# autonomousvision/unimatch

Measured on NVIDIA H100. Metric: image-pairs/sec @480x832 gmflow-scale2-refine6; EPE vs reference, higher is better.
Workload: dtype fp32

## Files before the change

### unimatch_b200/csrc/um_attention_tc.cu

```cuda
#include <math_constants.h>

#include "um_common.cuh"
#include "um_tc.cuh"

namespace um {

using namespace tc;

namespace {

constexpr int BM = 128, BN = 64;
constexpr int NTHREADS = 288;
constexpr int PRODUCER = 8;
constexpr uint32_t Q_BYTES = 4 * 16384;
constexpr uint32_t KV_STAGE_BYTES = 4 * 8192;
constexpr uint32_t OFF_Q = 0;
constexpr uint32_t OFF_K = OFF_Q + Q_BYTES;
constexpr uint32_t OFF_V = OFF_K + 2 * KV_STAGE_BYTES;
constexpr uint32_t OFF_X = OFF_V + 2 * KV_STAGE_BYTES;
constexpr uint32_t OFF_BAR = OFF_X + 1024;
constexpr uint32_t OFF_KREG = OFF_BAR + 256;
constexpr int MAX_LP = 2048;
constexpr uint32_t SMEM_BYTES = OFF_KREG + MAX_LP;
constexpr float SQRT_C = 11.313708498984761f;
constexpr float EXP_SCALE = 1.4426950408889634f / 11.313708498984761f;
constexpr float LAZY_THRESH = 8.0f / EXP_SCALE;

struct TcParams {
  float* out; long long ldo;
  int n_streams, kv_shift, lp;
  Geom g;
  const float* values; int vdim, value_mode, post_op;
  __half* out_split; long long split_plane;
};

__device__ __forceinline__ uint32_t pack_h2(__half a, __half b) {
  return (uint32_t)__half_as_ushort(a) | ((uint32_t)__half_as_ushort(b) << 16);
}

template <bool HAS_V>
__global__ void __launch_bounds__(NTHREADS, 1)
attn_tc_kernel(const __grid_constant__ CUtensorMap map_q, const __grid_constant__ CUtensorMap map_k,
               const __grid_constant__ CUtensorMap map_v, TcParams p) {
  extern __shared__ __align__(1024) uint8_t smem[];
  uint64_t* bars = reinterpret_cast<uint64_t*>(smem + OFF_BAR);
  uint64_t* q_full = bars + 0;
  uint64_t* k_full = bars + 1;
  uint64_t* k_empty = bars + 3;
  uint64_t* v_full = bars + 5;
  uint64_t* v_empty = bars + 7;
  int8_t* kreg = reinterpret_cast<int8_t*>(smem + OFF_KREG);

  const Geom g = p.g;
  const int warp = threadIdx.x >> 5, lane = threadIdx.x & 31;
  const int m0 = blockIdx.x * BM, win = blockIdx.y, n = blockIdx.z;
  const int nk = (n + p.kv_shift) % p.n_streams;
  const int nwin = g.nwin, lp = p.lp;
  const int T = (g.lw + BN - 1) / BN;
  const int planes = p.n_streams * nwin * lp;

  if (threadIdx.x == 0) {
    mbar_init(q_full, 1);
    for (int i = 0; i < 2; ++i) {
      mbar_init(k_full + i, 1); mbar_init(k_empty + i, 8);
      mbar_init(v_full + i, 1); mbar_init(v_empty + i, 8);
    }
    fence_barrier_init();
  }
  if (warp == PRODUCER && lane == 0) { tma_prefetch_desc(&map_q); tma_prefetch_desc(&map_k); tma_prefetch_desc(&map_v); }
  bool masked = false;
  if (g.mask_mode == UM_MASK_SWIN) {
    const int wy = win / g.kw, wx = win - wy * g.kw;
    masked = (g.sh > 0 && wy == g.kh - 1) || (g.sw > 0 && wx == g.kw - 1);
    if (masked)
      for (int t = threadIdx.x; t < g.lw; t += NTHREADS) {
        int yr, xr;
        window_token(g, win, t, &yr, &xr);
        kreg[t] = (int8_t)shift_region(g, yr, xr);
      }
  }
  __syncthreads();

  if (warp == PRODUCER) {
    const int qrow = (n * nwin + win) * lp + m0;
    if (elect_one()) {
      mbar_arrive_expect_tx(q_full, Q_BYTES);
#pragma unroll
      for (int part = 0; part < 2; ++part)
#pragma unroll
        for (int half = 0; half < 2; ++half)
          tma_load_2d(smem + OFF_Q + (part * 2 + half) * 16384, &map_q, q_full, half * 64, part * planes + qrow);
    }
    __syncwarp();
    const int krow = (nk * nwin + win) * lp;
    auto load_tile = [&](int j, const CUtensorMap* map, uint32_t off, uint64_t* full, uint64_t* empty) {
      const int s = j & 1;
      mbar_wait_inline(empty + s, ((j >> 1) & 1) ^ 1);
      if (elect_one()) {
        mbar_arrive_expect_tx(full + s, KV_STAGE_BYTES);
#pragma unroll
        for (int part = 0; part < 2; ++part)
#pragma unroll
          for (int half = 0; half < 2; ++half)
            tma_load_2d(smem + off + s * KV_STAGE_BYTES + (part * 2 + half) * 8192, map, full + s, half * 64,
                        part * planes + krow + j * BN);
      }
      __syncwarp();
    };
    load_tile(0, &map_k, OFF_K, k_full, k_empty);
    for (int j = 0; j < T; ++j) {
      if (j + 1 < T) load_tile(j + 1, &map_k, OFF_K, k_full, k_empty);
      if (HAS_V) load_tile(j, &map_v, OFF_V, v_full, v_empty);
    }
    return;
  }

  const int cw = warp;
  const int wg = cw >> 2;
  const int fr = wg * 64 + (cw & 3) * 16 + (lane >> 2);
  const int fc = 2 * (lane & 3);
  int rq[2] = {0, 0}, tok[2];
  bool row_valid[2];
#pragma unroll
  for (int h = 0; h < 2; ++h) {
    const int tq = m0 + fr + 8 * h;
    row_valid[h] = tq < g.lw;
    int yr = 0, xr = 0;
    tok[h] = row_valid[h] ? window_token(g, win, tq, &yr, &xr) : -1;
    if (masked) rq[h] = shift_region(g, yr, xr);
  }
  float m_run[2] = {-CUDART_INF_F, -CUDART_INF_F}, l_run[2] = {0.f, 0.f};
  const uint32_t q_base = smem_u32(smem + OFF_Q) + wg * 8192;
  auto consumers_sync = [&]() { asm volatile("bar.sync 1, 256;" ::: "memory"); };

  auto compute_s = [&](int j, float (&sv)[32]) {
    const int s = j & 1;
    mbar_wait_inline(k_full + s, (j >> 1) & 1);
    const uint32_t k_base = smem_u32(smem + OFF_K + s * KV_STAGE_BYTES);
    const int qa[3] = {1, 0, 0}, kb[3] = {0, 1, 0};
    fence_acc(sv);
    wgmma_fence();
#pragma unroll
    for (int c = 0; c < 3; ++c)
#pragma unroll
      for (int half = 0; half < 2; ++half)
#pragma unroll
        for (int ks = 0; ks < 4; ++ks)
          wgmma_ss<BN>(sv, desc_kmajor(q_base + (qa[c] * 2 + half) * 16384 + ks * 32),
                       desc_kmajor(k_base + (kb[c] * 2 + half) * 8192 + ks * 32), (c | half | ks) != 0);
    wgmma_commit();
    wgmma_wait<0>();
    fence_acc(sv);
    __syncwarp();
    if (lane == 0) mbar_arrive(k_empty + s);
  };
  mbar_wait_inline(q_full, 0);

  if (!HAS_V) {
    float* vals = reinterpret_cast<float*>(smem + OFF_X);
    const int et = threadIdx.x;
    const long long L = (long long)g.h * g.w;
    float a0[2] = {0.f, 0.f}, a1[2] = {0.f, 0.f};
    for (int j = 0; j < T; ++j) {
      const int s = j & 1;
      const int n0 = j * BN;
      if (et < BN) {
        float v0 = 0.f, v1 = 0.f;
        const int t = n0 + et;
        if (t < g.lw) {
          const int ktok = window_token(g, win, t);
          if (p.value_mode == UM_VALUE_TENSOR) {
            const float* vp = p.values + ((long long)nk * L + ktok) * p.vdim;
            v0 = __ldg(vp); v1 = (p.vdim > 1) ? __ldg(vp + 1) : 0.f;
          } else {
            const int ky = ktok / g.w;
            v0 = (float)(ktok - ky * g.w); v1 = (float)ky;
          }
        }
        vals[(s * BN + et) * 2] = v0; vals[(s * BN + et) * 2 + 1] = v1;
      }
      float sv[32];
      compute_s(j, sv);
      consumers_sync();
      const float2* vv = reinterpret_cast<const float2*>(vals + s * BN * 2);
#pragma unroll
      for (int h = 0; h < 2; ++h) {
        float mx = -CUDART_INF_F;
#pragma unroll
        for (int jj = 0; jj < 8; ++jj)
#pragma unroll
          for (int e = 0; e < 2; ++e) {
            float& x = sv[4 * jj + 2 * h + e];
            if (n0 + 8 * jj + fc + e >= g.lw) x = -CUDART_INF_F;
            mx = fmaxf(mx, x);
          }
        mx = fmaxf(mx, __shfl_xor_sync(0xffffffffu, mx, 1));
        mx = fmaxf(mx, __shfl_xor_sync(0xffffffffu, mx, 2));
        const float m_new = fmaxf(m_run[h], mx);
        const float alpha = exp2f((m_run[h] - m_new) * EXP_SCALE);
        m_run[h] = m_new;
        const float mscaled = m_new * EXP_SCALE;
        float sum = 0.f, b0 = 0.f, b1 = 0.f;
#pragma unroll
        for (int jj = 0; jj < 8; ++jj)
#pragma unroll
          for (int e = 0; e < 2; ++e) {
            const float pe = ex2_approx(fmaf(sv[4 * jj + 2 * h + e], EXP_SCALE, -mscaled));
            const float2 kv = vv[8 * jj + fc + e];
            sum += pe;
            b0 = fmaf(pe, kv.x, b0);
            b1 = fmaf(pe, kv.y, b1);
          }
        l_run[h] = l_run[h] * alpha + sum;
        a0[h] = a0[h] * alpha + b0;
        a1[h] = a1[h] * alpha + b1;
      }
    }
#pragma unroll
    for (int h = 0; h < 2; ++h) {
#pragma unroll
      for (int o = 1; o <= 2; o <<= 1) {
        l_run[h] += __shfl_xor_sync(0xffffffffu, l_run[h], o);
        a0[h] += __shfl_xor_sync(0xffffffffu, a0[h], o);
        a1[h] += __shfl_xor_sync(0xffffffffu, a1[h], o);
      }
      if (row_valid[h] && (lane & 3) == 0) {
        float r0 = a0[h] / l_run[h], r1 = a1[h] / l_run[h];
        const int oy = tok[h] / g.w, ox = tok[h] - oy * g.w;
        if (p.post_op == UM_POST_MINUS_OWN) { r0 -= (float)ox; r1 -= (float)oy; }
        else if (p.post_op == UM_POST_OWN_MINUS) { r0 = (float)ox - r0; }
        float* dst = p.out + ((long long)n * L + tok[h]) * p.vdim;
        dst[0] = r0;
        if (p.vdim > 1) dst[1] = r1;
      }
    }
    return;
  }

  float o[64];
#pragma unroll
  for (int i = 0; i < 64; ++i) o[i] = 0.f;
  for (int j = 0; j < T; ++j) {
    const int s = j & 1;
    const int n0 = j * BN;
    float sv[32];
    compute_s(j, sv);
    uint32_t ph[16], pl[16];
#pragma unroll
    for (int h = 0; h < 2; ++h) {
#pragma unroll
      for (int jj = 0; jj < 8; ++jj)
#pragma unroll
        for (int e = 0; e < 2; ++e) {
          const int col = n0 + 8 * jj + fc + e;
          float& x = sv[4 * jj + 2 * h + e];
          if (masked && kreg[col < g.lw ? col : 0] != rq[h]) x -= 100.0f * SQRT_C;
          if (col >= g.lw) x = -CUDART_INF_F;
        }
      float mx = -CUDART_INF_F;
#pragma unroll
      for (int jj = 0; jj < 8; ++jj) mx = fmaxf(mx, fmaxf(sv[4 * jj + 2 * h], sv[4 * jj + 2 * h + 1]));
      mx = fmaxf(mx, __shfl_xor_sync(0xffffffffu, mx, 1));
      mx = fmaxf(mx, __shfl_xor_sync(0xffffffffu, mx, 2));
      float alpha = 1.0f;
      if (mx > m_run[h] + LAZY_THRESH) {
        alpha = exp2f((m_run[h] - mx) * EXP_SCALE);
        m_run[h] = mx;
#pragma unroll
        for (int jj = 0; jj < 16; ++jj) { o[4 * jj + 2 * h] *= alpha; o[4 * jj + 2 * h + 1] *= alpha; }
      }
      const float mscaled = m_run[h] * EXP_SCALE;
      float sum = 0.f;
#pragma unroll
      for (int jj = 0; jj < 8; ++jj) {
        const float p0 = ex2_approx(fmaf(sv[4 * jj + 2 * h], EXP_SCALE, -mscaled));
        const float p1 = ex2_approx(fmaf(sv[4 * jj + 2 * h + 1], EXP_SCALE, -mscaled));
        sum += p0 + p1;
        split_f16x2(p0, p1, &ph[2 * jj + h], &pl[2 * jj + h]);
      }
      l_run[h] = l_run[h] * alpha + sum;
    }
    mbar_wait_inline(v_full + s, (j >> 1) & 1);
    const uint32_t v_base = smem_u32(smem + OFF_V + s * KV_STAGE_BYTES);
    fence_acc(o);
    wgmma_fence();
#pragma unroll
    for (int c = 0; c < 3; ++c)
#pragma unroll
      for (int ks = 0; ks < 4; ++ks) {
        const uint32_t* pp = c == 0 ? pl : ph;
        const uint32_t a[4] = {pp[4 * ks], pp[4 * ks + 1], pp[4 * ks + 2], pp[4 * ks + 3]};
        wgmma_rs_n128_tb(o, a, desc_mnmajor(v_base + (c == 1 ? 16384 : 0) + ks * 2048, 8192), true);
      }
    wgmma_commit();
    wgmma_wait<0>();
    fence_acc(o);
    __syncwarp();
    if (lane == 0) mbar_arrive(v_empty + s);
  }

  float inv[2];
#pragma unroll
  for (int h = 0; h < 2; ++h) {
    float l = l_run[h];
    l += __shfl_xor_sync(0xffffffffu, l, 1);
    l += __shfl_xor_sync(0xffffffffu, l, 2);
    inv[h] = 1.0f / l;
  }
  consumers_sync();
  float* osm = reinterpret_cast<float*>(smem + OFF_Q);
#pragma unroll
  for (int jj = 0; jj < 16; ++jj)
#pragma unroll
    for (int h = 0; h < 2; ++h) {
      const int row = fr + 8 * h, col = 8 * jj + fc;
      *reinterpret_cast<float2*>(osm + row * 128 + (((col >> 2) ^ (row & 31)) << 2) + (col & 3)) =
          make_float2(o[4 * jj + 2 * h] * inv[h], o[4 * jj + 2 * h + 1] * inv[h]);
    }
  consumers_sync();
  float* obase = p.out + (long long)n * g.h * g.w * p.ldo;
  for (int row = cw * 16; row < cw * 16 + 16; ++row) {
    const int tq = m0 + row;
    if (tq >= g.lw) break;
    const int tk = window_token(g, win, tq);
    const float4 v = *reinterpret_cast<const float4*>(osm + row * 128 + ((lane ^ (row & 31)) << 2));
    if (p.out) *reinterpret_cast<float4*>(obase + (long long)tk * p.ldo + lane * 4) = v;
    if (p.out_split) {
      uint32_t h0, h1, l0, l1;
      split_f16x2(v.x, v.y, &h0, &l0);
      split_f16x2(v.z, v.w, &h1, &l1);
      __half* d = p.out_split + ((long long)n * g.h * g.w + tk) * 128 + lane * 4;
      *reinterpret_cast<uint2*>(d) = make_uint2(h0, h1);
      *reinterpret_cast<uint2*>(d + p.split_plane) = make_uint2(l0, l1);
    }
  }
}

struct SplitParams {
  const float* src[3]; long long ld[3];
  __half* dst[3];
  int n_streams, lp;
  Geom g;
};

__global__ void __launch_bounds__(256) split_windows_kernel(SplitParams p) {
  const Geom g = p.g;
  const int lane = threadIdx.x & 31;
  const int t = blockIdx.x * 8 + (threadIdx.x >> 5);
  const int win = blockIdx.y, n = blockIdx.z;
  if (t >= p.lp) return;
  const long long planes = (long long)p.n_streams * g.nwin * p.lp;
  const long long row = ((long long)n * g.nwin + win) * p.lp + t;
  const int tok = (t < g.lw) ? window_token(g, win, t) : -1;
#pragma unroll
  for (int a = 0; a < 3; ++a) {
    if (!p.src[a]) continue;
    float4 x = make_float4(0.f, 0.f, 0.f, 0.f);
    if (tok >= 0) x = __ldg(reinterpret_cast<const float4*>(p.src[a] + ((long long)n * g.h * g.w + tok) * p.ld[a]) + lane);
// ... 60 lines not shown
  sp.src[0] = q; sp.src[1] = k; sp.src[2] = v;
  sp.ld[0] = ldq; sp.ld[1] = ldk; sp.ld[2] = ldv;
  sp.dst[0] = wq; sp.dst[1] = wk; sp.dst[2] = wv;
  sp.n_streams = n_streams; sp.lp = padded_lw(g.lw); sp.g = g;
  split_windows_kernel<<<dim3((sp.lp + 7) / 8, g.nwin, n_streams), 256, 0, st>>>(sp);
  return check_launch(what);
}


int attention_planes_launch(const __half* wq, const __half* wk, const __half* wv, float* out, long long ldo, __half* out_split,
                               long long split_plane, int n_streams, int kv_shift, const Geom& g, cudaStream_t st) {
  const int lp = padded_lw(g.lw);
  int rc;
  CUtensorMap mq, mk, mv;
  const uint64_t rows = (uint64_t)2 * n_streams * g.nwin * lp;
  if ((rc = make_map_2d_f16(&mq, wq, rows, 128, BM))) return rc;
  if ((rc = make_map_2d_f16(&mk, wk, rows, 128, BN))) return rc;
  if ((rc = make_map_2d_f16(&mv, wv, rows, 128, BN))) return rc;
  static PerDeviceBytes configured;
  if ((rc = ensure_smem(configured, attn_tc_kernel<true>, SMEM_BYTES, "attn_tc"))) return rc;
  TcParams p{};
  p.out = out; p.ldo = ldo; p.n_streams = n_streams; p.kv_shift = kv_shift; p.lp = lp; p.g = g;
  p.out_split = out_split; p.split_plane = split_plane;
  const int qtiles = (g.lw + BM - 1) / BM;
  attn_tc_kernel<true><<<dim3(qtiles, g.nwin, n_streams), NTHREADS, SMEM_BYTES, st>>>(mq, mk, mv, p);
  return check_launch("um_window_attention(wgmma)");
}

int window_attention_tc(const float* q, const float* k, const float* v, float* out, int n_streams, int kv_shift,
                        long long ldq, long long ldk, long long ldv, long long ldo, const Geom& g, void* workspace,
                        cudaStream_t st) {
  const int lp = padded_lw(g.lw);
  const size_t plane_elems = (size_t)2 * n_streams * g.nwin * lp * 128;
  __half* wq = reinterpret_cast<__half*>(workspace);
  __half* wk = wq + plane_elems;
  __half* wv = wk + plane_elems;
  int rc = split_windows_launch(q, k, v, ldq, ldk, ldv, wq, wk, wv, n_streams, g, st, "um_window_attention(split)");
  if (rc) return rc;
  return attention_planes_launch(wq, wk, wv, out, ldo, nullptr, 0, n_streams, kv_shift, g, st);
}

int softmax_expectation_tc(const float* q, const float* k, const float* values, float* out, int n_streams, int n_total,
                           int kv_shift, long long ldq, long long ldk, int vdim, int value_mode, int post_op,
                           const Geom& g, void* workspace, cudaStream_t st) {
  const int lp = padded_lw(g.lw);
  const size_t plane_elems = (size_t)2 * n_total * g.nwin * lp * 128;
  __half* wq = reinterpret_cast<__half*>(workspace);
  __half* wk = wq + plane_elems;
  int rc = split_windows_launch(q, k, nullptr, ldq, ldk, 0, wq, wk, nullptr, n_total, g, st, "um_softmax_expectation(split)");
  if (rc) return rc;
  CUtensorMap mq, mk;
  const uint64_t rows = (uint64_t)2 * n_total * g.nwin * lp;
  if ((rc = make_map_2d_f16(&mq, wq, rows, 128, BM))) return rc;
  if ((rc = make_map_2d_f16(&mk, wk, rows, 128, BN))) return rc;
  static PerDeviceBytes configured;
  if ((rc = ensure_smem(configured, attn_tc_kernel<false>, SMEM_BYTES, "expect_tc"))) return rc;
  TcParams p{};
  p.out = out; p.ldo = vdim; p.n_streams = n_total; p.kv_shift = kv_shift; p.lp = lp; p.g = g;
  p.values = values; p.vdim = vdim; p.value_mode = value_mode; p.post_op = post_op;
  const int qtiles = (g.lw + BM - 1) / BM;
  attn_tc_kernel<false><<<dim3(qtiles, g.nwin, n_streams), NTHREADS, SMEM_BYTES, st>>>(mq, mk, mk, p);
  return check_launch("um_softmax_expectation(wgmma)");
}

}
```

### unimatch_b200/csrc/um_tc.cuh

```cuda
#pragma once
#include <cuda.h>
#include <cuda_fp16.h>
#include <cuda_runtime.h>
#include <stdint.h>

namespace um {
namespace tc {

__device__ __forceinline__ uint32_t smem_u32(const void* p) { return (uint32_t)__cvta_generic_to_shared(p); }

__device__ __forceinline__ bool elect_one() {
  uint32_t pred = 0;
  asm volatile(
      "{\n\t.reg .pred P;\n\telect.sync _|P, 0xffffffff;\n\tselp.u32 %0, 1, 0, P;\n\t}\n"
      : "=r"(pred));
  return pred != 0;
}

__device__ __forceinline__ void mbar_init(uint64_t* bar, uint32_t count) {
  asm volatile("mbarrier.init.shared::cta.b64 [%0], %1;" ::"r"(smem_u32(bar)), "r"(count));
}
__device__ __forceinline__ void fence_barrier_init() { asm volatile("fence.mbarrier_init.release.cluster;" ::: "memory"); }
__device__ __forceinline__ void fence_proxy_async() { asm volatile("fence.proxy.async.shared::cta;" ::: "memory"); }
__device__ __forceinline__ void mbar_arrive(uint64_t* bar) {
  asm volatile("mbarrier.arrive.shared::cta.b64 _, [%0];" ::"r"(smem_u32(bar)) : "memory");
}
__device__ __forceinline__ void mbar_arrive_expect_tx(uint64_t* bar, uint32_t bytes) {
  asm volatile("mbarrier.arrive.expect_tx.shared::cta.b64 _, [%0], %1;" ::"r"(smem_u32(bar)), "r"(bytes) : "memory");
}
__device__ __forceinline__ bool mbar_try_wait(uint64_t* bar, uint32_t parity) {
  uint32_t ok;
  asm volatile(
      "{\n\t.reg .pred P;\n\tmbarrier.try_wait.parity.shared::cta.b64 P, [%1], %2;\n\tselp.u32 %0, 1, 0, P;\n\t}\n"
      : "=r"(ok)
      : "r"(smem_u32(bar)), "r"(parity)
      : "memory");
  return ok != 0;
}
static __device__ __noinline__ void mbar_wait_slow(uint64_t* bar, uint32_t parity) {
#pragma unroll 1
  for (uint32_t i = 0; i < (1u << 22); ++i)
    if (mbar_try_wait(bar, parity)) return;
  printf("um::tc mbarrier timeout: block (%d,%d,%d) thread %d bar %p parity %u\n", blockIdx.x, blockIdx.y, blockIdx.z,
         threadIdx.x, (void*)bar, parity);
  __trap();
}
__device__ __forceinline__ void mbar_wait(uint64_t* bar, uint32_t parity) {
  if (!mbar_try_wait(bar, parity)) mbar_wait_slow(bar, parity);
}
__device__ __forceinline__ void mbar_wait_inline(uint64_t* bar, uint32_t parity) {
#pragma unroll 1
// ... 38 lines not shown
__device__ __forceinline__ uint64_t desc_kmajor(uint32_t saddr) { return smem_desc_sw128(saddr, 16, 1024); }
__device__ __forceinline__ uint64_t desc_mnmajor(uint32_t saddr, uint32_t mn_group_stride) {
  return smem_desc_sw128(saddr, mn_group_stride, 1024);
}

template <int N>
__device__ __forceinline__ void setmaxnreg_inc() { asm volatile("setmaxnreg.inc.sync.aligned.u32 %0;" ::"n"(N)); }
template <int N>
__device__ __forceinline__ void setmaxnreg_dec() { asm volatile("setmaxnreg.dec.sync.aligned.u32 %0;" ::"n"(N)); }

__device__ __forceinline__ void wgmma_fence() { asm volatile("wgmma.fence.sync.aligned;" ::: "memory"); }
__device__ __forceinline__ void wgmma_commit() { asm volatile("wgmma.commit_group.sync.aligned;" ::: "memory"); }
template <int N>
__device__ __forceinline__ void wgmma_wait() { asm volatile("wgmma.wait_group.sync.aligned %0;" ::"n"(N) : "memory"); }
template <int N>
__device__ __forceinline__ void fence_acc(float (&d)[N]) {
#pragma unroll
  for (int i = 0; i < N; ++i) asm volatile("" : "+f"(d[i])::"memory");
}

template <int N>
__device__ __forceinline__ void wgmma_ss(float (&d)[N / 2], uint64_t da, uint64_t db, bool accumulate);
template <>
__device__ __forceinline__ void wgmma_ss<16>(float (&d)[8], uint64_t da, uint64_t db, bool accumulate) {
  asm volatile(
      "{\n\t.reg .pred p;\n\tsetp.ne.b32 p, %10, 0;\n\t"
      "wgmma.mma_async.sync.aligned.m64n16k16.f32.f16.f16 {%0, %1, %2, %3, %4, %5, %6, %7}, %8, %9, p, 1, 1, 0, 0;\n\t}\n"
      : "+f"(d[0]), "+f"(d[1]), "+f"(d[2]), "+f"(d[3]), "+f"(d[4]), "+f"(d[5]), "+f"(d[6]), "+f"(d[7])
      : "l"(da), "l"(db), "r"((uint32_t)accumulate));
}
template <>
__device__ __forceinline__ void wgmma_ss<64>(float (&d)[32], uint64_t da, uint64_t db, bool accumulate) {
  asm volatile(
      "{\n\t.reg .pred p;\n\tsetp.ne.b32 p, %34, 0;\n\t"
      "wgmma.mma_async.sync.aligned.m64n64k16.f32.f16.f16 {%0, %1, %2, %3, %4, %5, %6, %7, %8, %9, %10, %11, %12, %13, %14, %15, %16, %17, %18, %19, %20, %21, %22, %23, %24, %25, %26, %27, %28, %29, %30, %31}, %32, %33, p, 1, 1, 0, 0;\n\t}\n"
      : "+f"(d[0]), "+f"(d[1]), "+f"(d[2]), "+f"(d[3]), "+f"(d[4]), "+f"(d[5]), "+f"(d[6]), "+f"(d[7]), "+f"(d[8]), "+f"(d[9]), "+f"(d[10]), "+f"(d[11]), "+f"(d[12]), "+f"(d[13]), "+f"(d[14]), "+f"(d[15]), "+f"(d[16]), "+f"(d[17]), "+f"(d[18]), "+f"(d[19]), "+f"(d[20]), "+f"(d[21]), "+f"(d[22]), "+f"(d[23]), "+f"(d[24]), "+f"(d[25]), "+f"(d[26]), "+f"(d[27]), "+f"(d[28]), "+f"(d[29]), "+f"(d[30]), "+f"(d[31])
      : "l"(da), "l"(db), "r"((uint32_t)accumulate));
}
template <>
__device__ __forceinline__ void wgmma_ss<96>(float (&d)[48], uint64_t da, uint64_t db, bool accumulate) {
  asm volatile(
      "{\n\t.reg .pred p;\n\tsetp.ne.b32 p, %50, 0;\n\t"
      "wgmma.mma_async.sync.aligned.m64n96k16.f32.f16.f16 {%0, %1, %2, %3, %4, %5, %6, %7, %8, %9, %10, %11, %12, %13, %14, %15, %16, %17, %18, %19, %20, %21, %22, %23, %24, %25, %26, %27, %28, %29, %30, %31, %32, %33, %34, %35, %36, %37, %38, %39, %40, %41, %42, %43, %44, %45, %46, %47}, %48, %49, p, 1, 1, 0, 0;\n\t}\n"
      : "+f"(d[0]), "+f"(d[1]), "+f"(d[2]), "+f"(d[3]), "+f"(d[4]), "+f"(d[5]), "+f"(d[6]), "+f"(d[7]), "+f"(d[8]), "+f"(d[9]), "+f"(d[10]), "+f"(d[11]), "+f"(d[12]), "+f"(d[13]), "+f"(d[14]), "+f"(d[15]), "+f"(d[16]), "+f"(d[17]), "+f"(d[18]), "+f"(d[19]), "+f"(d[20]), "+f"(d[21]), "+f"(d[22]), "+f"(d[23]), "+f"(d[24]), "+f"(d[25]), "+f"(d[26]), "+f"(d[27]), "+f"(d[28]), "+f"(d[29]), "+f"(d[30]), "+f"(d[31]), "+f"(d[32]), "+f"(d[33]), "+f"(d[34]), "+f"(d[35]), "+f"(d[36]), "+f"(d[37]), "+f"(d[38]), "+f"(d[39]), "+f"(d[40]), "+f"(d[41]), "+f"(d[42]), "+f"(d[43]), "+f"(d[44]), "+f"(d[45]), "+f"(d[46]), "+f"(d[47])
      : "l"(da), "l"(db), "r"((uint32_t)accumulate));
}
template <>
__device__ __forceinline__ void wgmma_ss<128>(float (&d)[64], uint64_t da, uint64_t db, bool accumulate) {
  asm volatile(
      "{\n\t.reg .pred p;\n\tsetp.ne.b32 p, %66, 0;\n\t"
      "wgmma.mma_async.sync.aligned.m64n128k16.f32.f16.f16 {%0, %1, %2, %3, %4, %5, %6, %7, %8, %9, %10, %11, %12, %13, %14, %15, %16, %17, %18, %19, %20, %21, %22, %23, %24, %25, %26, %27, %28, %29, %30, %31, %32, %33, %34, %35, %36, %37, %38, %39, %40, %41, %42, %43, %44, %45, %46, %47, %48, %49, %50, %51, %52, %53, %54, %55, %56, %57, %58, %59, %60, %61, %62, %63}, %64, %65, p, 1, 1, 0, 0;\n\t}\n"
// ... 70 lines not shown
```

Measured before the change: 82.32.

## Make wgmma window attention persistent with warpgroup ping-pong and tail-sized MMAs

Converts the attention kernels into persistent kernels. Each CTA loops over (stream, window, q-tile) work items with a rotated tile order and reloads Q through a q_full/q_empty barrier pair, while the producer computes the shift-mask region table into a double buffer. In the value-tensor path the two consumer warpgroups alternate turns through named barriers (ping-pong) so one group's softmax overlaps the other's MMAs. The last partial key tile uses narrower wgmma shapes (n8/n16/n32) sized to the tail. Output is written directly from registers instead of being staged through shared memory, trading coalesced stores for less synchronisation, and the added scheduling complexity risks barrier-phase bugs.

```diff
diff --git a/unimatch_b200/csrc/um_attention_tc.cu b/unimatch_b200/csrc/um_attention_tc.cu
--- a/unimatch_b200/csrc/um_attention_tc.cu
+++ b/unimatch_b200/csrc/um_attention_tc.cu
@@ -1,4 +1,6 @@
 #include <math_constants.h>
+
+#include <type_traits>
 
 #include "um_common.cuh"
 #include "um_tc.cuh"
@@ -21,7 +23,7 @@
 constexpr uint32_t OFF_BAR = OFF_X + 1024;
 constexpr uint32_t OFF_KREG = OFF_BAR + 256;
 constexpr int MAX_LP = 2048;
-constexpr uint32_t SMEM_BYTES = OFF_KREG + MAX_LP;
+constexpr uint32_t SMEM_BYTES = OFF_KREG + 2 * MAX_LP;
 constexpr float SQRT_C = 11.313708498984761f;
 constexpr float EXP_SCALE = 1.4426950408889634f / 11.313708498984761f;
 constexpr float LAZY_THRESH = 8.0f / EXP_SCALE;
@@ -29,6 +31,7 @@
 struct TcParams {
   float* out; long long ldo;
   int n_streams, kv_shift, lp;
+  int qtiles, n_items;
   Geom g;
   const float* values; int vdim, value_mode, post_op;
   __half* out_split; long long split_plane;
@@ -36,6 +39,25 @@
 
 __device__ __forceinline__ uint32_t pack_h2(__half a, __half b) {
   return (uint32_t)__half_as_ushort(a) | ((uint32_t)__half_as_ushort(b) << 16);
+}
+
+struct Item {
+  int n, win, m0;
+};
+__device__ __forceinline__ Item decode_item(const TcParams& p, int item) {
+  const int grp = item / p.qtiles;
+  int qt = item - grp * p.qtiles + grp % p.qtiles;
+  if (qt >= p.qtiles) qt -= p.qtiles;
+  Item r;
+  r.n = grp / p.g.nwin;
+  r.win = grp - r.n * p.g.nwin;
+  r.m0 = qt * BM;
+  return r;
+}
+__device__ __forceinline__ bool window_masked(const Geom& g, int win) {
+  if (g.mask_mode != UM_MASK_SWIN) return false;
+  const int wy = win / g.kw, wx = win - wy * g.kw;
+  return (g.sh > 0 && wy == g.kh - 1) || (g.sw > 0 && wx == g.kw - 1);
 }
 
 template <bool HAS_V>
@@ -45,22 +67,20 @@
   extern __shared__ __align__(1024) uint8_t smem[];
   uint64_t* bars = reinterpret_cast<uint64_t*>(smem + OFF_BAR);
   uint64_t* q_full = bars + 0;
-  uint64_t* k_full = bars + 1;
-  uint64_t* k_empty = bars + 3;
-  uint64_t* v_full = bars + 5;
-  uint64_t* v_empty = bars + 7;
-  int8_t* kreg = reinterpret_cast<int8_t*>(smem + OFF_KREG);
+  uint64_t* q_empty = bars + 1;
+  uint64_t* k_full = bars + 2;
+  uint64_t* k_empty = bars + 4;
+  uint64_t* v_full = bars + 6;
+  uint64_t* v_empty = bars + 8;
 
   const Geom g = p.g;
   const int warp = threadIdx.x >> 5, lane = threadIdx.x & 31;
-  const int m0 = blockIdx.x * BM, win = blockIdx.y, n = blockIdx.z;
-  const int nk = (n + p.kv_shift) % p.n_streams;
   const int nwin = g.nwin, lp = p.lp;
   const int T = (g.lw + BN - 1) / BN;
   const int planes = p.n_streams * nwin * lp;
 
   if (threadIdx.x == 0) {
-    mbar_init(q_full, 1);
+    mbar_init(q_full, 32); mbar_init(q_empty, 8);
     for (int i = 0; i < 2; ++i) {
       mbar_init(k_full + i, 1); mbar_init(k_empty + i, 8);
       mbar_init(v_full + i, 1); mbar_init(v_empty + i, 8);
@@ -68,34 +88,13 @@
     fence_barrier_init();
   }
   if (warp == PRODUCER && lane == 0) { tma_prefetch_desc(&map_q); tma_prefetch_desc(&map_k); tma_prefetch_desc(&map_v); }
-  bool masked = false;
-  if (g.mask_mode == UM_MASK_SWIN) {
-    const int wy = win / g.kw, wx = win - wy * g.kw;
-    masked = (g.sh > 0 && wy == g.kh - 1) || (g.sw > 0 && wx == g.kw - 1);
-    if (masked)
-      for (int t = threadIdx.x; t < g.lw; t += NTHREADS) {
-        int yr, xr;
-        window_token(g, win, t, &yr, &xr);
-        kreg[t] = (int8_t)shift_region(g, yr, xr);
-      }
-  }
   __syncthreads();
 
   if (warp == PRODUCER) {
-    const int qrow = (n * nwin + win) * lp + m0;
-    if (elect_one()) {
-      mbar_arrive_expect_tx(q_full, Q_BYTES);
-#pragma unroll
-      for (int part = 0; part < 2; ++part)
-#pragma unroll
-        for (int half = 0; half < 2; ++half)
-          tma_load_2d(smem + OFF_Q + (part * 2 + half) * 16384, &map_q, q_full, half * 64, part * planes + qrow);
-    }
-    __syncwarp();
-    const int krow = (nk * nwin + win) * lp;
-    auto load_tile = [&](int j, const CUtensorMap* map, uint32_t off, uint64_t* full, uint64_t* empty) {
-      const int s = j & 1;
-      mbar_wait_inline(empty + s, ((j >> 1) & 1) ^ 1);
+    uint32_t kc = 0, vc = 0;
+    auto load_tile = [&](uint32_t& c, int row, const CUtensorMap* map, uint32_t off, uint64_t* full, uint64_t* empty) {
+      const int s = c & 1;
+      mbar_wait_inline(empty + s, ((c >> 1) & 1) ^ 1);
       if (elect_one()) {
         mbar_arrive_expect_tx(full + s, KV_STAGE_BYTES);
 #pragma unroll
@@ -103,237 +102,334 @@
 #pragma unroll
           for (int half = 0; half < 2; ++half)
             tma_load_2d(smem + off + s * KV_STAGE_BYTES + (part * 2 + half) * 8192, map, full + s, half * 64,
-                        part * planes + krow + j * BN);
+                        part * planes + row);
       }
       __syncwarp();
+      ++c;
     };
-    load_tile(0, &map_k, OFF_K, k_full, k_empty);
-    for (int j = 0; j < T; ++j) {
-      if (j + 1 < T) load_tile(j + 1, &map_k, OFF_K, k_full, k_empty);
-      if (HAS_V) load_tile(j, &map_v, OFF_V, v_full, v_empty);
+    int it = 0;
+    for (int item = blockIdx.x; item < p.n_items; item += gridDim.x, ++it) {
+      const Item t = decode_item(p, item);
+      const int nk = (t.n + p.kv_shift) % p.n_streams;
+      const int krow = (nk * nwin + t.win) * lp;
+      load_tile(kc, krow, &map_k, OFF_K, k_full, k_empty);
+      mbar_wait_inline(q_empty, (it & 1) ^ 1);
+      const int qrow = (t.n * nwin + t.win) * lp + t.m0;
+      if (elect_one()) {
+        mbar_expect_tx(q_full, Q_BYTES);
+#pragma unroll
+        for (int part = 0; part < 2; ++part)
+#pragma unroll
+          for (int half = 0; half < 2; ++half)
+            tma_load_2d(smem + OFF_Q + (part * 2 + half) * 16384, &map_q, q_full, half * 64, part * planes + qrow);
+      }
+      __syncwarp();
+      if (HAS_V && window_masked(g, t.win)) {
+        int8_t* kreg = reinterpret_cast<int8_t*>(smem + OFF_KREG) + (it & 1) * MAX_LP;
+        for (int k = lane; k < g.lw; k += 32) {
+          int yr, xr;
+          window_token(g, t.win, k, &yr, &xr);
+          kreg[k] = (int8_t)shift_region(g, yr, xr);
+        }
+      }
+      mbar_arrive(q_full);
+      for (int j = 0; j < T; ++j) {
+        if (j + 1 < T) load_tile(kc, krow + (j + 1) * BN, &map_k, OFF_K, k_full, k_empty);
+        if (HAS_V) load_tile(vc, krow + j * BN, &map_v, OFF_V, v_full, v_empty);
+      }
     }
     return;
   }
 
   const int cw = warp;
-  const int wg = cw >> 2;
+  const int wg = __shfl_sync(0xffffffffu, cw >> 2, 0);
   const int fr = wg * 64 + (cw & 3) * 16 + (lane >> 2);
   const int fc = 2 * (lane & 3);
+  const uint32_t q_base = smem_u32(smem + OFF_Q) + wg * 8192;
+  const int tail = g.lw - (T - 1) * BN;
+
+  auto issue_s = [&](auto width, uint32_t k_base, float (&sv)[32]) {
+    constexpr int N = decltype(width)::value;
+    float(&d)[N / 2] = *reinterpret_cast<float(*)[N / 2]>(&sv);
+    const int qa[3] = {1, 0, 0}, kb[3] = {0, 1, 0};
+#pragma unroll
+    for (int c = 0; c < 3; ++c)
+#pragma unroll
+      for (int half = 0; half < 2; ++half)
+#pragma unroll
+        for (int ks = 0; ks < 4; ++ks)
+          wgmma_ss<N>(d, desc_kmajor(q_base + (qa[c] * 2 + half) * 16384 + ks * 32),
+                      desc_kmajor(k_base + (kb[c] * 2 + half) * 8192 + ks * 32), (c | half | ks) != 0);
+  };
+  float m_run[2], l_run[2];
   int rq[2] = {0, 0}, tok[2];
   bool row_valid[2];
-#pragma unroll
-  for (int h = 0; h < 2; ++h) {
-    const int tq = m0 + fr + 8 * h;
-    row_valid[h] = tq < g.lw;
-    int yr = 0, xr = 0;
-    tok[h] = row_valid[h] ? window_token(g, win, tq, &yr, &xr) : -1;
-    if (masked) rq[h] = shift_region(g, yr, xr);
-  }
-  float m_run[2] = {-CUDART_INF_F, -CUDART_INF_F}, l_run[2] = {0.f, 0.f};
-  const uint32_t q_base = smem_u32(smem + OFF_Q) + wg * 8192;
-  auto consumers_sync = [&]() { asm volatile("bar.sync 1, 256;" ::: "memory"); };
-
-  auto compute_s = [&](int j, float (&sv)[32]) {
-    const int s = j & 1;
-    mbar_wait_inline(k_full + s, (j >> 1) & 1);
-    const uint32_t k_base = smem_u32(smem + OFF_K + s * KV_STAGE_BYTES);
-    const int qa[3] = {1, 0, 0}, kb[3] = {0, 1, 0};
-    fence_acc(sv);
-    wgmma_fence();
-#pragma unroll
-    for (int c = 0; c < 3; ++c)
-#pragma unroll
-      for (int half = 0; half < 2; ++half)
-#pragma unroll
-        for (int ks = 0; ks < 4; ++ks)
-          wgmma_ss<BN>(sv, desc_kmajor(q_base + (qa[c] * 2 + half) * 16384 + ks * 32),
-                       desc_kmajor(k_base + (kb[c] * 2 + half) * 8192 + ks * 32), (c | half | ks) != 0);
-    wgmma_commit();
-    wgmma_wait<0>();
-    fence_acc(sv);
-    __syncwarp();
-    if (lane == 0) mbar_arrive(k_empty + s);
-  };
-  mbar_wait_inline(q_full, 0);
+  uint32_t kc = 0, vc = 0;
+  int it = 0;
 
   if (!HAS_V) {
     float* vals = reinterpret_cast<float*>(smem + OFF_X);
     const int et = threadIdx.x;
     const long long L = (long long)g.h * g.w;
-    float a0[2] = {0.f, 0.f}, a1[2] = {0.f, 0.f};
-    for (int j = 0; j < T; ++j) {
-      const int s = j & 1;
-      const int n0 = j * BN;
-      if (et < BN) {
-        float v0 = 0.f, v1 = 0.f;
-        const int t = n0 + et;
-        if (t < g.lw) {
-          const int ktok = window_token(g, win, t);
-          if (p.value_mode == UM_VALUE_TENSOR) {
-            const float* vp = p.values + ((long long)nk * L + ktok) * p.vdim;
-            v0 = __ldg(vp); v1 = (p.vdim > 1) ? __ldg(vp + 1) : 0.f;
-          } else {
-            const int ky = ktok / g.w;
-            v0 = (float)(ktok - ky * g.w); v1 = (float)ky;
+    for (int item = blockIdx.x; item < p.n_items; item += gridDim.x, ++it) {
+      const Item t = decode_item(p, item);
+      const int nk = (t.n + p.kv_shift) % p.n_streams;
+#pragma unroll
+      for (int h = 0; h < 2; ++h) {
+        const int tq = t.m0 + fr + 8 * h;
+        row_valid[h] = tq < g.lw;
+        tok[h] = row_valid[h] ? window_token(g, t.win, tq) : -1;
+        m_run[h] = -CUDART_INF_F; l_run[h] = 0.f;
+      }
+      float a0[2] = {0.f, 0.f}, a1[2] = {0.f, 0.f};
+      mbar_wait_inline(q_full, it & 1);
+      for (int j = 0; j < T; ++j) {
+        const int s = kc & 1;
+        const int n0 = j * BN;
+        if (et < BN) {
+          float v0 = 0.f, v1 = 0.f;
+          const int tk = n0 + et;
+          if (tk < g.lw) {
+            const int ktok = window_token(g, t.win, tk);
+            if (p.value_mode == UM_VALUE_TENSOR) {
+              const float* vp = p.values + ((long long)nk * L + ktok) * p.vdim;
+              v0 = __ldg(vp); v1 = (p.vdim > 1) ? __ldg(vp + 1) : 0.f;
+            } else {
+              const int ky = ktok / g.w;
+              v0 = (float)(ktok - ky * g.w); v1 = (float)ky;
+            }
           }
-        }
-        vals[(s * BN + et) * 2] = v0; vals[(s * BN + et) * 2 + 1] = v1;
-      }
-      float sv[32];
-      compute_s(j, sv);
-      consumers_sync();
-      const float2* vv = reinterpret_cast<const float2*>(vals + s * BN * 2);
+          vals[(s * BN + et) * 2] = v0; vals[(s * BN + et) * 2 + 1] = v1;
+        }
+        float sv[32];
+        mbar_wait_inline(k_full + s, (kc >> 1) & 1);
+        fence_acc(sv);
+        wgmma_fence();
+        issue_s(std::integral_constant<int, BN>{}, smem_u32(smem + OFF_K + s * KV_STAGE_BYTES), sv);
+        wgmma_commit();
+        wgmma_wait<0>();
+        fence_acc(sv);
+        __syncwarp();
+        if (lane == 0) {
+          mbar_arrive(k_empty + s);
+          if (j == T - 1) mbar_arrive(q_empty);
+        }
+        ++kc;
+        asm volatile("bar.sync 1, 256;" ::: "memory");
+        const float2* vv = reinterpret_cast<const float2*>(vals + s * BN * 2);
+#pragma unroll
+        for (int h = 0; h < 2; ++h) {
+          float mx = -CUDART_INF_F;
+#pragma unroll
+          for (int jj = 0; jj < 8; ++jj)
+#pragma unroll
+            for (int e = 0; e < 2; ++e) {
+              float& x = sv[4 * jj + 2 * h + e];
+              if (n0 + 8 * jj + fc + e >= g.lw) x = -CUDART_INF_F;
+              mx = fmaxf(mx, x);
+            }
+          mx = fmaxf(mx, __shfl_xor_sync(0xffffffffu, mx, 1));
+          mx = fmaxf(mx, __shfl_xor_sync(0xffffffffu, mx, 2));
+          const float m_new = fmaxf(m_run[h], mx);
+          const float alpha = exp2f((m_run[h] - m_new) * EXP_SCALE);
+          m_run[h] = m_new;
+          const float mscaled = m_new * EXP_SCALE;
+          float sum = 0.f, b0 = 0.f, b1 = 0.f;
+#pragma unroll
+          for (int jj = 0; jj < 8; ++jj)
+#pragma unroll
+            for (int e = 0; e < 2; ++e) {
+              const float pe = ex2_approx(fmaf(sv[4 * jj + 2 * h + e], EXP_SCALE, -mscaled));
+              const float2 kv = vv[8 * jj + fc + e];
+              sum += pe;
+              b0 = fmaf(pe, kv.x, b0);
+              b1 = fmaf(pe, kv.y, b1);
+            }
+          l_run[h] = l_run[h] * alpha + sum;
+          a0[h] = a0[h] * alpha + b0;
+          a1[h] = a1[h] * alpha + b1;
+        }
+      }
 #pragma unroll
       for (int h = 0; h < 2; ++h) {
-        float mx = -CUDART_INF_F;
-#pragma unroll
-        for (int jj = 0; jj < 8; ++jj)
-#pragma unroll
-          for (int e = 0; e < 2; ++e) {
-            float& x = sv[4 * jj + 2 * h + e];
-            if (n0 + 8 * jj + fc + e >= g.lw) x = -CUDART_INF_F;
-            mx = fmaxf(mx, x);
-          }
-        mx = fmaxf(mx, __shfl_xor_sync(0xffffffffu, mx, 1));
-        mx = fmaxf(mx, __shfl_xor_sync(0xffffffffu, mx, 2));
-        const float m_new = fmaxf(m_run[h], mx);
-        const float alpha = exp2f((m_run[h] - m_new) * EXP_SCALE);
-        m_run[h] = m_new;
-        const float mscaled = m_new * EXP_SCALE;
-        float sum = 0.f, b0 = 0.f, b1 = 0.f;
-#pragma unroll
-        for (int jj = 0; jj < 8; ++jj)
-#pragma unroll
-          for (int e = 0; e < 2; ++e) {
-            const float pe = ex2_approx(fmaf(sv[4 * jj + 2 * h + e], EXP_SCALE, -mscaled));
-            const float2 kv = vv[8 * jj + fc + e];
-            sum += pe;
-            b0 = fmaf(pe, kv.x, b0);
-            b1 = fmaf(pe, kv.y, b1);
-          }
-        l_run[h] = l_run[h] * alpha + sum;
-        a0[h] = a0[h] * alpha + b0;
-        a1[h] = a1[h] * alpha + b1;
-      }
-    }
-#pragma unroll
-    for (int h = 0; h < 2; ++h) {
-#pragma unroll
-      for (int o = 1; o <= 2; o <<= 1) {
-        l_run[h] += __shfl_xor_sync(0xffffffffu, l_run[h], o);
-        a0[h] += __shfl_xor_sync(0xffffffffu, a0[h], o);
-        a1[h] += __shfl_xor_sync(0xffffffffu, a1[h], o);
-      }
-      if (row_valid[h] && (lane & 3) == 0) {
-        float r0 = a0[h] / l_run[h], r1 = a1[h] / l_run[h];
-        const int oy = tok[h] / g.w, ox = tok[h] - oy * g.w;
-        if (p.post_op == UM_POST_MINUS_OWN) { r0 -= (float)ox; r1 -= (float)oy; }
-        else if (p.post_op == UM_POST_OWN_MINUS) { r0 = (float)ox - r0; }
-        float* dst = p.out + ((long long)n * L + tok[h]) * p.vdim;
-        dst[0] = r0;
-        if (p.vdim > 1) dst[1] = r1;
+#pragma unroll
+        for (int o = 1; o <= 2; o <<= 1) {
+          l_run[h] += __shfl_xor_sync(0xffffffffu, l_run[h], o);
+          a0[h] += __shfl_xor_sync(0xffffffffu, a0[h], o);
+          a1[h] += __shfl_xor_sync(0xffffffffu, a1[h], o);
+        }
+        if (row_valid[h] && (lane & 3) == 0) {
+          float r0 = a0[h] / l_run[h], r1 = a1[h] / l_run[h];
+          const int oy = tok[h] / g.w, ox = tok[h] - oy * g.w;
+          if (p.post_op == UM_POST_MINUS_OWN) { r0 -= (float)ox; r1 -= (float)oy; }
+          else if (p.post_op == UM_POST_OWN_MINUS) { r0 = (float)ox - r0; }
+          float* dst = p.out + ((long long)t.n * L + tok[h]) * p.vdim;
+          dst[0] = r0;
+          if (p.vdim > 1) dst[1] = r1;
+        }
       }
     }
     return;
   }
 
+  auto turn_wait = [&]() {
+    if (wg == 0) asm volatile("bar.sync 2, 256;" ::: "memory");
+    else asm volatile("bar.sync 3, 256;" ::: "memory");
+  };
+  auto turn_pass = [&]() {
+    if (wg == 0) asm volatile("bar.arrive 3, 256;" ::: "memory");
+    else asm volatile("bar.arrive 2, 256;" ::: "memory");
+  };
+  if (wg == 1) turn_pass();
   float o[64];
-#pragma unroll
-  for (int i = 0; i < 64; ++i) o[i] = 0.f;
-  for (int j = 0; j < T; ++j) {
-    const int s = j & 1;
-    const int n0 = j * BN;
-    float sv[32];
-    compute_s(j, sv);
-    uint32_t ph[16], pl[16];
-#pragma unroll
-    for (int h = 0; h < 2; ++h) {
-#pragma unroll
-      for (int jj = 0; jj < 8; ++jj)
-#pragma unroll
-        for (int e = 0; e < 2; ++e) {
-          const int col = n0 + 8 * jj + fc + e;
-          float& x = sv[4 * jj + 2 * h + e];
-          if (masked && kreg[col < g.lw ? col : 0] != rq[h]) x -= 100.0f * SQRT_C;
-          if (col >= g.lw) x = -CUDART_INF_F;
-        }
-      float mx = -CUDART_INF_F;
-#pragma unroll
-      for (int jj = 0; jj < 8; ++jj) mx = fmaxf(mx, fmaxf(sv[4 * jj + 2 * h], sv[4 * jj + 2 * h + 1]));
-      mx = fmaxf(mx, __shfl_xor_sync(0xffffffffu, mx, 1));
-      mx = fmaxf(mx, __shfl_xor_sync(0xffffffffu, mx, 2));
-      float alpha = 1.0f;
-      if (mx > m_run[h] + LAZY_THRESH) {
-        alpha = exp2f((m_run[h] - mx) * EXP_SCALE);
-        m_run[h] = mx;
-#pragma unroll
-        for (int jj = 0; jj < 16; ++jj) { o[4 * jj + 2 * h] *= alpha; o[4 * jj + 2 * h + 1] *= alpha; }
-      }
-      const float mscaled = m_run[h] * EXP_SCALE;
-      float sum = 0.f;
-#pragma unroll
-      for (int jj = 0; jj < 8; ++jj) {
-        const float p0 = ex2_approx(fmaf(sv[4 * jj + 2 * h], EXP_SCALE, -mscaled));
-        const float p1 = ex2_approx(fmaf(sv[4 * jj + 2 * h + 1], EXP_SCALE, -mscaled));
-        sum += p0 + p1;
-        split_f16x2(p0, p1, &ph[2 * jj + h], &pl[2 * jj + h]);
-      }
-      l_run[h] = l_run[h] * alpha + sum;
-    }
-    mbar_wait_inline(v_full + s, (j >> 1) & 1);
-    const uint32_t v_base = smem_u32(smem + OFF_V + s * KV_STAGE_BYTES);
-    fence_acc(o);
-    wgmma_fence();
+  float sv[32];
+  uint32_t ph[16], pl[16];
+  auto issue_pv = [&](auto steps, uint32_t v_base) {
+    constexpr int NKS = decltype(steps)::value;
 #pragma unroll
     for (int c = 0; c < 3; ++c)
 #pragma unroll
-      for (int ks = 0; ks < 4; ++ks) {
+      for (int ks = 0; ks < NKS; ++ks) {
         const uint32_t* pp = c == 0 ? pl : ph;
         const uint32_t a[4] = {pp[4 * ks], pp[4 * ks + 1], pp[4 * ks + 2], pp[4 * ks + 3]};
         wgmma_rs_n128_tb(o, a, desc_mnmajor(v_base + (c == 1 ? 16384 : 0) + ks * 2048, 8192), true);
       }
-    wgmma_commit();
-    wgmma_wait<0>();
-    fence_acc(o);
-    __syncwarp();
-    if (lane == 0) mbar_arrive(v_empty + s);
+  };
+  const int8_t* kreg_base = reinterpret_cast<const int8_t*>(smem + OFF_KREG);
+  for (int item = blockIdx.x; item < p.n_items; item += gridDim.x, ++it) {
+    const Item t = decode_item(p, item);
+    const bool masked = window_masked(g, t.win);
+    const int8_t* kreg = kreg_base + (it & 1) * MAX_LP;
+    const bool active = t.m0 + wg * 64 < g.lw;
+#pragma unroll
+    for (int h = 0; h < 2; ++h) {
+      const int tq = t.m0 + fr + 8 * h;
+      row_valid[h] = tq < g.lw;
+      int yr = 0, xr = 0;
+      tok[h] = row_valid[h] ? window_token(g, t.win, tq, &yr, &xr) : -1;
+      rq[h] = masked ? shift_region(g, yr, xr) : 0;
+      m_run[h] = -CUDART_INF_F; l_run[h] = 0.f;
+    }
+#pragma unroll
+    for (int i = 0; i < 64; ++i) o[i] = 0.f;
+    mbar_wait_inline(q_full, it & 1);
+    for (int j = 0; j <= T; ++j) {
+      const bool do_pv = j > 0, do_s = j < T;
+      const int sk = kc & 1, svs = vc & 1;
+      turn_wait();
+      if (active) {
+        if (do_pv) mbar_wait_inline(v_full + svs, (vc >> 1) & 1);
+        if (do_s) mbar_wait_inline(k_full + sk, (kc >> 1) & 1);
+        const uint32_t v_base = smem_u32(smem + OFF_V + svs * KV_STAGE_BYTES);
+        const uint32_t k_base = smem_u32(smem + OFF_K + sk * KV_STAGE_BYTES);
+        auto stage = [&](auto pv_steps, auto s_width) {
+          fence_acc(o);
+          fence_acc(sv);
+          wgmma_fence();
+          if constexpr (decltype(pv_steps)::value > 0) issue_pv(pv_steps, v_base);
+          if constexpr (decltype(s_width)::value > 0) issue_s(s_width, k_base, sv);
+          wgmma_commit();
+          turn_pass();
+          wgmma_wait<0>();
+          fence_acc(o);
+          fence_acc(sv);
+        };
+        using I0 = std::integral_constant<int, 0>;
+        using P4 = std::integral_constant<int, 4>;
+        using S64 = std::integral_constant<int, BN>;
+        if (j == 0) stage(I0{}, S64{});
+        else if (j < T - 1 || (j == T - 1 && tail > 32)) stage(P4{}, S64{});
+        else if (j == T - 1) {
+          if (tail > 16) stage(P4{}, std::integral_constant<int, 32>{});
+          else if (tail > 8) stage(P4{}, std::integral_constant<int, 16>{});
+          else stage(P4{}, std::integral_constant<int, 8>{});
+        } else {
+          if (tail > 48) stage(P4{}, I0{});
+          else if (tail > 32) stage(std::integral_constant<int, 3>{}, I0{});
+          else if (tail > 16) stage(std::integral_constant<int, 2>{}, I0{});
+          else stage(std::integral_constant<int, 1>{}, I0{});
+        }
+      } else {
+        turn_pass();
+        if (do_pv) mbar_wait_inline(v_full + svs, (vc >> 1) & 1);
+        if (do_s) mbar_wait_inline(k_full + sk, (kc >> 1) & 1);
+      }
+      __syncwarp();
+      if (lane == 0) {
+        if (do_pv) mbar_arrive(v_empty + svs);
+        if (do_s) mbar_arrive(k_empty + sk);
+        if (j == T - 1) mbar_arrive(q_empty);
+      }
+      vc += do_pv;
+      kc += do_s;
+      if (!active || !do_s) continue;
+      const int n0 = j * BN;
+#pragma unroll
+      for (int h = 0; h < 2; ++h) {
+#pragma unroll
+        for (int jj = 0; jj < 8; ++jj)
+#pragma unroll
+          for (int e = 0; e < 2; ++e) {
+            const int col = n0 + 8 * jj + fc + e;
+            float& x = sv[4 * jj + 2 * h + e];
+            if (masked && kreg[col < g.lw ? col : 0] != rq[h]) x -= 100.0f * SQRT_C;
+            if (col >= g.lw) x = -CUDART_INF_F;
+          }
+        float mx = -CUDART_INF_F;
+#pragma unroll
+        for (int jj = 0; jj < 8; ++jj) mx = fmaxf(mx, fmaxf(sv[4 * jj + 2 * h], sv[4 * jj + 2 * h + 1]));
+        mx = fmaxf(mx, __shfl_xor_sync(0xffffffffu, mx, 1));
+        mx = fmaxf(mx, __shfl_xor_sync(0xffffffffu, mx, 2));
+        float alpha = 1.0f;
+        if (mx > m_run[h] + LAZY_THRESH) {
+          alpha = exp2f((m_run[h] - mx) * EXP_SCALE);
+          m_run[h] = mx;
+#pragma unroll
+          for (int jj = 0; jj < 16; ++jj) { o[4 * jj + 2 * h] *= alpha; o[4 * jj + 2 * h + 1] *= alpha; }
+        }
+        const float mscaled = m_run[h] * EXP_SCALE;
+        float sum = 0.f;
+#pragma unroll
+        for (int jj = 0; jj < 8; ++jj) {
+          const float p0 = ex2_approx(fmaf(sv[4 * jj + 2 * h], EXP_SCALE, -mscaled));
+          const float p1 = ex2_approx(fmaf(sv[4 * jj + 2 * h + 1], EXP_SCALE, -mscaled));
+          sum += p0 + p1;
+          split_f16x2(p0, p1, &ph[2 * jj + h], &pl[2 * jj + h]);
+        }
+        l_run[h] = l_run[h] * alpha + sum;
+      }
+    }
+    if (!active) continue;
+
+    float inv[2];
+#pragma unroll
+    for (int h = 0; h < 2; ++h) {
+      float l = l_run[h];
+      l += __shfl_xor_sync(0xffffffffu, l, 1);
+      l += __shfl_xor_sync(0xffffffffu, l, 2);
+      inv[h] = 1.0f / l;
+    }
+    const long long row0 = (long long)t.n * g.h * g.w;
+#pragma unroll
+    for (int h = 0; h < 2; ++h) {
+      if (!row_valid[h]) continue;
+      float* orow = p.out ? p.out + (row0 + tok[h]) * p.ldo : nullptr;
+      __half* srow = p.out_split ? p.out_split + (row0 + tok[h]) * 128 : nullptr;
+#pragma unroll
+      for (int jj = 0; jj < 16; ++jj) {
+        const int col = 8 * jj + fc;
+        const float v0 = o[4 * jj + 2 * h] * inv[h], v1 = o[4 * jj + 2 * h + 1] * inv[h];
+        if (orow) *reinterpret_cast<float2*>(orow + col) = make_float2(v0, v1);
+        if (srow) {
+          uint32_t hi, lo;
+          split_f16x2(v0, v1, &hi, &lo);
+          *reinterpret_cast<uint32_t*>(srow + col) = hi;
+          *reinterpret_cast<uint32_t*>(srow + p.split_plane + col) = lo;
+        }
+      }
+    }
   }
-
-  float inv[2];
-#pragma unroll
-  for (int h = 0; h < 2; ++h) {
-    float l = l_run[h];
-    l += __shfl_xor_sync(0xffffffffu, l, 1);
-    l += __shfl_xor_sync(0xffffffffu, l, 2);
-    inv[h] = 1.0f / l;
-  }
-  consumers_sync();
-  float* osm = reinterpret_cast<float*>(smem + OFF_Q);
-#pragma unroll
-  for (int jj = 0; jj < 16; ++jj)
-#pragma unroll
-    for (int h = 0; h < 2; ++h) {
-      const int row = fr + 8 * h, col = 8 * jj + fc;
-      *reinterpret_cast<float2*>(osm + row * 128 + (((col >> 2) ^ (row & 31)) << 2) + (col & 3)) =
-          make_float2(o[4 * jj + 2 * h] * inv[h], o[4 * jj + 2 * h + 1] * inv[h]);
-    }
-  consumers_sync();
-  float* obase = p.out + (long long)n * g.h * g.w * p.ldo;
-  for (int row = cw * 16; row < cw * 16 + 16; ++row) {
-    const int tq = m0 + row;
-    if (tq >= g.lw) break;
-    const int tk = window_token(g, win, tq);
-    const float4 v = *reinterpret_cast<const float4*>(osm + row * 128 + ((lane ^ (row & 31)) << 2));
-    if (p.out) *reinterpret_cast<float4*>(obase + (long long)tk * p.ldo + lane * 4) = v;
-    if (p.out_split) {
-      uint32_t h0, h1, l0, l1;
-      split_f16x2(v.x, v.y, &h0, &l0);
-      split_f16x2(v.z, v.w, &h1, &l1);
-      __half* d = p.out_split + ((long long)n * g.h * g.w + tk) * 128 + lane * 4;
-      *reinterpret_cast<uint2*>(d) = make_uint2(h0, h1);
-      *reinterpret_cast<uint2*>(d + p.split_plane) = make_uint2(l0, l1);
-    }
-  }
+  if (wg == 0) turn_wait();
 }
 
 struct SplitParams {
@@ -440,8 +536,10 @@
   TcParams p{};
   p.out = out; p.ldo = ldo; p.n_streams = n_streams; p.kv_shift = kv_shift; p.lp = lp; p.g = g;
   p.out_split = out_split; p.split_plane = split_plane;
-  const int qtiles = (g.lw + BM - 1) / BM;
-  attn_tc_kernel<true><<<dim3(qtiles, g.nwin, n_streams), NTHREADS, SMEM_BYTES, st>>>(mq, mk, mv, p);
+  p.qtiles = (g.lw + BM - 1) / BM;
+  p.n_items = p.qtiles * g.nwin * n_streams;
+  const int grid = p.n_items < device_sm_count() ? p.n_items : device_sm_count();
+  attn_tc_kernel<true><<<grid, NTHREADS, SMEM_BYTES, st>>>(mq, mk, mv, p);
   return check_launch("um_window_attention(wgmma)");
 }
 
@@ -476,8 +574,10 @@
   TcParams p{};
   p.out = out; p.ldo = vdim; p.n_streams = n_total; p.kv_shift = kv_shift; p.lp = lp; p.g = g;
   p.values = values; p.vdim = vdim; p.value_mode = value_mode; p.post_op = post_op;
-  const int qtiles = (g.lw + BM - 1) / BM;
-  attn_tc_kernel<false><<<dim3(qtiles, g.nwin, n_streams), NTHREADS, SMEM_BYTES, st>>>(mq, mk, mk, p);
+  p.qtiles = (g.lw + BM - 1) / BM;
+  p.n_items = p.qtiles * g.nwin * n_streams;
+  const int grid = p.n_items < device_sm_count() ? p.n_items : device_sm_count();
+  attn_tc_kernel<false><<<grid, NTHREADS, SMEM_BYTES, st>>>(mq, mk, mk, p);
   return check_launch("um_softmax_expectation(wgmma)");
 }
 
diff --git a/unimatch_b200/csrc/um_tc.cuh b/unimatch_b200/csrc/um_tc.cuh
--- a/unimatch_b200/csrc/um_tc.cuh
+++ b/unimatch_b200/csrc/um_tc.cuh
@@ -27,6 +27,9 @@
 }
 __device__ __forceinline__ void mbar_arrive_expect_tx(uint64_t* bar, uint32_t bytes) {
   asm volatile("mbarrier.arrive.expect_tx.shared::cta.b64 _, [%0], %1;" ::"r"(smem_u32(bar)), "r"(bytes) : "memory");
+}
+__device__ __forceinline__ void mbar_expect_tx(uint64_t* bar, uint32_t bytes) {
+  asm volatile("mbarrier.expect_tx.relaxed.cta.shared::cta.b64 [%0], %1;" ::"r"(smem_u32(bar)), "r"(bytes) : "memory");
 }
 __device__ __forceinline__ bool mbar_try_wait(uint64_t* bar, uint32_t parity) {
   uint32_t ok;
@@ -111,11 +114,27 @@
 template <int N>
 __device__ __forceinline__ void wgmma_ss(float (&d)[N / 2], uint64_t da, uint64_t db, bool accumulate);
 template <>
+__device__ __forceinline__ void wgmma_ss<8>(float (&d)[4], uint64_t da, uint64_t db, bool accumulate) {
+  asm volatile(
+      "{\n\t.reg .pred p;\n\tsetp.ne.b32 p, %6, 0;\n\t"
+      "wgmma.mma_async.sync.aligned.m64n8k16.f32.f16.f16 {%0, %1, %2, %3}, %4, %5, p, 1, 1, 0, 0;\n\t}\n"
+      : "+f"(d[0]), "+f"(d[1]), "+f"(d[2]), "+f"(d[3])
+      : "l"(da), "l"(db), "r"((uint32_t)accumulate));
+}
+template <>
 __device__ __forceinline__ void wgmma_ss<16>(float (&d)[8], uint64_t da, uint64_t db, bool accumulate) {
   asm volatile(
       "{\n\t.reg .pred p;\n\tsetp.ne.b32 p, %10, 0;\n\t"
       "wgmma.mma_async.sync.aligned.m64n16k16.f32.f16.f16 {%0, %1, %2, %3, %4, %5, %6, %7}, %8, %9, p, 1, 1, 0, 0;\n\t}\n"
       : "+f"(d[0]), "+f"(d[1]), "+f"(d[2]), "+f"(d[3]), "+f"(d[4]), "+f"(d[5]), "+f"(d[6]), "+f"(d[7])
+      : "l"(da), "l"(db), "r"((uint32_t)accumulate));
+}
+template <>
+__device__ __forceinline__ void wgmma_ss<32>(float (&d)[16], uint64_t da, uint64_t db, bool accumulate) {
+  asm volatile(
+      "{\n\t.reg .pred p;\n\tsetp.ne.b32 p, %18, 0;\n\t"
+      "wgmma.mma_async.sync.aligned.m64n32k16.f32.f16.f16 {%0, %1, %2, %3, %4, %5, %6, %7, %8, %9, %10, %11, %12, %13, %14, %15}, %16, %17, p, 1, 1, 0, 0;\n\t}\n"
+      : "+f"(d[0]), "+f"(d[1]), "+f"(d[2]), "+f"(d[3]), "+f"(d[4]), "+f"(d[5]), "+f"(d[6]), "+f"(d[7]), "+f"(d[8]), "+f"(d[9]), "+f"(d[10]), "+f"(d[11]), "+f"(d[12]), "+f"(d[13]), "+f"(d[14]), "+f"(d[15])
       : "l"(da), "l"(db), "r"((uint32_t)accumulate));
 }
 template <>
```

New measurement: 83.16, median of 6. 1.01x the previous value.
